# danijar/embodied

Hardware: AMD Instinct MI355X
Metric: env steps/sec + learner train-steps/sec, 64 envs 84x84x4 obs, 1/2/4/8 GPU (higher is better)
Workload: dtype u8

## Files before the change

### embodied_amd/csrc/device_util.h

```cpp
#pragma once

#include "kernels.h"

#include <cstdint>

namespace emb {
namespace {

typedef unsigned int u32x4 __attribute__((ext_vector_type(4)));

typedef __attribute__((address_space(1))) u32x4 gu32x4;
template <bool kNonTemporal>
__device__ __forceinline__ u32x4 load16(const u32x4* p) {
  const gu32x4* g = (const gu32x4*)p;
  if constexpr (kNonTemporal) return __builtin_nontemporal_load(g);
  else return *g;
}
template <bool kNonTemporal>
__device__ __forceinline__ void store16(u32x4* p, u32x4 v) {
  gu32x4* g = (gu32x4*)p;
  if constexpr (kNonTemporal) __builtin_nontemporal_store(v, g);
  else *g = v;
}

constexpr int kThreads = 256;

template <typename T>
__device__ __forceinline__ T gload(const void* p) {
  return *(const __attribute__((address_space(1))) T*)p;
}
template <typename T>
__device__ __forceinline__ void gstore(void* p, T v) {
  *(__attribute__((address_space(1))) T*)p = v;
}

template <typename T>
__device__ __forceinline__ void copy_unit(const uint8_t* s, uint8_t* d) {
  gstore<T>(d, gload<T>(s));
}

typedef unsigned int u32x2_t __attribute__((ext_vector_type(2)));

__device__ __forceinline__ void copy_bytes(const uint8_t* s, uint8_t* d, int unit) {
  switch (unit) {
    case 16: copy_unit<u32x4>(s, d); break;
    case 8: copy_unit<u32x2_t>(s, d); break;
    case 4: copy_unit<uint32_t>(s, d); break;
    case 2: copy_unit<uint16_t>(s, d); break;
    default: copy_unit<uint8_t>(s, d); break;
  }
}

template <typename T>
__device__ __forceinline__ T put_masked(const uint8_t* src, uint8_t* pool, uint8_t* out, bool keep) {
  const T v = gload<T>(src) * static_cast<T>(keep ? 1 : 0);
  if (pool) gstore<T>(pool, v);
  if (out) gstore<T>(out, v);
  return v;
}

__device__ __forceinline__ uint16_t put_masked_bf16(const uint8_t* src, uint8_t* pool, uint8_t* out, bool keep) {
  const float x = __uint_as_float(static_cast<uint32_t>(gload<uint16_t>(src)) << 16);
  const uint16_t v = static_cast<uint16_t>(__float_as_uint(x * (keep ? 1.f : 0.f)) >> 16);
  if (pool) gstore<uint16_t>(pool, v);
  if (out) gstore<uint16_t>(out, v);
  return v;
}

template <typename T>
__device__ __forceinline__ uint64_t masked_bits(T v) {
  static_assert(sizeof(T) <= 8, "a masked element fits 64 bits");
  uint64_t bits = 0;
  __builtin_memcpy(&bits, &v, sizeof(T));
  return bits;
}

__device__ __forceinline__ uint64_t put_masked_as(int dtype, const uint8_t* src, uint8_t* pool, uint8_t* out,
                                                  bool keep) {
  switch (dtype) {
    case kU8: case kBool: return masked_bits(put_masked<uint8_t>(src, pool, out, keep));
    case kI8: return masked_bits(put_masked<int8_t>(src, pool, out, keep));
    case kI16: return masked_bits(put_masked<int16_t>(src, pool, out, keep));
    case kI32: return masked_bits(put_masked<int32_t>(src, pool, out, keep));
    case kI64: return masked_bits(put_masked<int64_t>(src, pool, out, keep));
    case kF16: return masked_bits(put_masked<_Float16>(src, pool, out, keep));
    case kBF16: return masked_bits(put_masked_bf16(src, pool, out, keep));
    case kF32: return masked_bits(put_masked<float>(src, pool, out, keep));
    default: return masked_bits(put_masked<double>(src, pool, out, keep));
  }
}

int dtype_size(int dtype) {
  switch (dtype) {
    case kU8: case kI8: case kBool: return 1;
    case kI16: case kF16: case kBF16: return 2;
    case kI32: case kF32: return 4;
    case kI64: case kF64: return 8;
    default: return 0;
  }
}

}
}
```

### embodied_amd/csrc/step.hip

```cpp
#include "device_util.h"

#include <hip/hip_bf16.h>
#include <hip/hip_fp16.h>
#include <hip/hip_ext.h>

#include <algorithm>
#include <cstddef>
#include <cstring>

namespace emb {
namespace {


template <typename Out>
__device__ __forceinline__ Out cvt(uint8_t v, float scale, float offset);
template <> __device__ __forceinline__ uint8_t cvt<uint8_t>(uint8_t v, float, float) { return v; }
template <> __device__ __forceinline__ float cvt<float>(uint8_t v, float s, float o) { return fmaf(static_cast<float>(v), s, o); }
template <> __device__ __forceinline__ __half cvt<__half>(uint8_t v, float s, float o) { return __float2half(fmaf(static_cast<float>(v), s, o)); }
template <> __device__ __forceinline__ __hip_bfloat16 cvt<__hip_bfloat16>(uint8_t v, float s, float o) { return __float2bfloat16(fmaf(static_cast<float>(v), s, o)); }

template <typename Out>
struct alignas(4 * sizeof(Out)) Quad { Out v[4]; };

typedef unsigned int u32x2 __attribute__((ext_vector_type(2)));

template <typename Out>
__device__ __forceinline__ void store_quad(Out* dst, const Quad<Out>& q) {
  if constexpr (sizeof(Quad<Out>) == 4) {
    uint32_t w;
    __builtin_memcpy(&w, &q, 4);
    __builtin_nontemporal_store(w, reinterpret_cast<uint32_t*>(dst));
  } else if constexpr (sizeof(Quad<Out>) == 8) {
    u32x2 w;
    __builtin_memcpy(&w, &q, 8);
    __builtin_nontemporal_store(w, reinterpret_cast<u32x2*>(dst));
  } else {
    u32x4 w;
    __builtin_memcpy(&w, &q, 16);
    __builtin_nontemporal_store(w, reinterpret_cast<u32x4*>(dst));
  }
}

template <typename Out, int C, bool kChannelsFirst>
__global__ __launch_bounds__(kThreads) void obs_stack_kernel(
    const uint8_t* src, const int32_t* env_ids, Out* dst, int64_t pixels,
    float scale, float offset) {
  const int64_t n = blockIdx.y;
  const int64_t e = env_ids ? env_ids[n] : n;
  const int64_t quads = pixels >> 2;
  const uint32_t* frame = reinterpret_cast<const uint32_t*>(src + e * pixels * C);
  Out* out = dst + n * pixels * C;
  for (int64_t q = static_cast<int64_t>(blockIdx.x) * kThreads + threadIdx.x; q < quads;
       q += static_cast<int64_t>(gridDim.x) * kThreads) {
    uint32_t w[C];
#pragma unroll
    for (int c = 0; c < C; ++c) w[c] = frame[q * C + c];
    auto byte_at = [&w](int idx) {
      return static_cast<uint8_t>((w[idx >> 2] >> ((idx & 3) * 8)) & 0xFFu);
    };
    if (kChannelsFirst) {
#pragma unroll
      for (int c = 0; c < C; ++c) {
        Quad<Out> o;
#pragma unroll
        for (int p = 0; p < 4; ++p) o.v[p] = cvt<Out>(byte_at(p * C + c), scale, offset);
        store_quad(out + c * pixels + q * 4, o);
      }
    } else {
#pragma unroll
      for (int j = 0; j < C; ++j) {
        Quad<Out> o;
#pragma unroll
        for (int p = 0; p < 4; ++p) o.v[p] = cvt<Out>(byte_at(j * 4 + p), scale, offset);
        store_quad(out + (q * C + j) * 4, o);
      }
    }
  }
}

template <typename Out>
__global__ __launch_bounds__(kThreads) void obs_stack_generic_kernel(
    const uint8_t* src, const int32_t* env_ids, Out* dst, int64_t pixels,
    int64_t channels, int layout, float scale, float offset) {
  const int64_t n = blockIdx.y;
  const int64_t e = env_ids ? env_ids[n] : n;
  const int64_t elems = pixels * channels;
  const uint8_t* frame = src + e * elems;
  Out* out = dst + n * elems;
  for (int64_t i = static_cast<int64_t>(blockIdx.x) * kThreads + threadIdx.x; i < elems;
       i += static_cast<int64_t>(gridDim.x) * kThreads) {
    int64_t s = i;
    if (layout == kLayoutChannelsFirst) {
      const int64_t c = i / pixels, p = i - c * pixels;
      s = p * channels + c;
    }
    out[i] = cvt<Out>(frame[s], scale, offset);
  }
}

template <typename Out>
hipError_t obs_stack_typed(const uint8_t* src, const int32_t* env_ids, void* dst,
                           int64_t n, int64_t pixels, int64_t channels, int layout,
                           float scale, float offset, hipStream_t stream) {
  Out* out = static_cast<Out*>(dst);
  const bool fast = pixels % 4 == 0 && channels >= 1 && channels <= 4 &&
                    reinterpret_cast<uint64_t>(src) % 4 == 0 &&
                    (pixels * channels) % 4 == 0 &&
                    reinterpret_cast<uint64_t>(dst) % (4 * sizeof(Out)) == 0;
  if (!fast) {
    const int64_t elems = pixels * channels;
    dim3 grid(static_cast<uint32_t>(std::min<int64_t>((elems + kThreads - 1) / kThreads, 64)),
              static_cast<uint32_t>(n));
    hipLaunchKernelGGL(obs_stack_generic_kernel<Out>, grid, dim3(kThreads), 0, stream,
                       src, env_ids, out, pixels, channels, layout, scale, offset);
    return hipGetLastError();
  }
  const int64_t quads = pixels / 4;
  dim3 grid(static_cast<uint32_t>(std::min<int64_t>((quads + kThreads - 1) / kThreads, 32)),
            static_cast<uint32_t>(n));
  const bool cf = layout == kLayoutChannelsFirst && channels > 1;
#define EMB_OBS(C)                                                                         \
  if (cf) hipLaunchKernelGGL((obs_stack_kernel<Out, C, true>), grid, dim3(kThreads), 0,   \
                             stream, src, env_ids, out, pixels, scale, offset);           \
  else hipLaunchKernelGGL((obs_stack_kernel<Out, C, false>), grid, dim3(kThreads), 0,     \
                          stream, src, env_ids, out, pixels, scale, offset);
  switch (channels) {
    case 1: EMB_OBS(1) break;
    case 2: EMB_OBS(2) break;
    case 3: EMB_OBS(3) break;
    default: EMB_OBS(4) break;
  }
#undef EMB_OBS
  return hipGetLastError();
}

struct PreKey {
  const uint8_t* src;
  uint8_t* pool;
  int64_t rowbytes;
};
struct PreCarry {
  const uint8_t* src;
  uint8_t* pool;
  const uint8_t* flags;
  int32_t rowbytes, dtype, elem, pad;
};
struct alignas(16) PreTable {
  uint8_t* stepid_pool;
  int32_t* rows_out;
  PreKey narrow[kPreNarrow];
  PreCarry carry;
  uint32_t words[1];
};
struct PrewriteArgs {
  const uint8_t* frames;
  void* dst;
  uint8_t* frame_pool;
  int32_t pixels, frame_blocks;
  float scale, offset;
  int32_t n, n_narrow;
  const PreTable* table;
};
static_assert(sizeof(PrewriteArgs) == 56, "obs_stack_insert_kernel's arguments (passed one by one) fit the 14 preloaded dwords");

__device__ __forceinline__ void prewrite_carry(const PreTable& t, const uint32_t* tab, int32_t n_envs,
                                               int64_t n) {
  const PreCarry c = t.carry;
  if (!c.src) return;
  const int64_t prev = static_cast<int32_t>(gload<uint32_t>(tab + 6 * static_cast<int64_t>(n_envs) + n));
  const int64_t off = static_cast<int64_t>(threadIdx.x) * c.elem;
  if (prev < 0 || off >= c.rowbytes) return;
  const bool keep = gload<uint8_t>(c.flags + prev) == 0;
  const uint8_t* src = c.src + n * c.rowbytes + off;
  uint8_t* pool = c.pool + prev * c.rowbytes + off;
  put_masked_as(c.dtype, src, pool, nullptr, keep);
}

__device__ __forceinline__ void prewrite_narrow(const PrewriteArgs& a, int64_t n) {
  const PreTable& t = *a.table;
  const uint32_t* tab = t.words;
  prewrite_carry(t, tab, a.n, n);
  const int64_t row = static_cast<int32_t>(gload<uint32_t>(tab + n));
  if (row < 0) return;
  uint32_t sid = 0;
  if (threadIdx.x < kStepBytes / 4)
    sid = gload<uint32_t>(tab + a.n + n * (kStepBytes / 4) + threadIdx.x);
  PreKey key[kPreNarrow];
#pragma unroll
  for (int k = 0; k < kPreNarrow; ++k) key[k] = t.narrow[k];
  uint8_t v[kPreNarrow];
#pragma unroll
  for (int k = 0; k < kPreNarrow; ++k) {
    v[k] = 0;
    if (k < a.n_narrow && static_cast<int64_t>(threadIdx.x) < key[k].rowbytes)
      v[k] = gload<uint8_t>(key[k].src + n * key[k].rowbytes + threadIdx.x);
  }
#pragma unroll
  for (int k = 0; k < kPreNarrow; ++k)
    if (k < a.n_narrow && static_cast<int64_t>(threadIdx.x) < key[k].rowbytes)
      gstore<uint8_t>(key[k].pool + row * key[k].rowbytes + threadIdx.x, v[k]);
  if (t.stepid_pool && threadIdx.x < kStepBytes / 4)
    gstore<uint32_t>(t.stepid_pool + row * kStepBytes + threadIdx.x * 4, sid);
  if (t.rows_out && threadIdx.x == 0) t.rows_out[n] = static_cast<int32_t>(row);
}
static_assert(kThreads >= 256, "a narrow key (<= 256 bytes per step) is one byte per lane");

template <typename Out, int C, bool kChannelsFirst>
__global__ __launch_bounds__(kThreads) void obs_stack_insert_kernel(
    const uint8_t* frames, const PreTable* table, uint8_t* frame_pool, void* dst,
    int32_t pixels_, int32_t frame_blocks, int32_t n_envs, int32_t n_narrow, float scale, float offset) {
  const PrewriteArgs a{frames, dst, frame_pool, pixels_, frame_blocks, scale, offset, n_envs, n_narrow, table};
  if (blockIdx.x < static_cast<uint32_t>(n_envs)) {
    prewrite_narrow(a, blockIdx.x);
    return;
  }
  const uint32_t id = blockIdx.x - static_cast<uint32_t>(n_envs);
  const int64_t n = id / static_cast<uint32_t>(frame_blocks);
  const uint32_t block = id - static_cast<uint32_t>(n) * static_cast<uint32_t>(frame_blocks);
  const int64_t pixels = a.pixels;
  const int64_t quads = pixels >> 2;
  const uint32_t* frame = reinterpret_cast<const uint32_t*>(a.frames + n * pixels * C);
  Out* out = static_cast<Out*>(a.dst) + n * pixels * C;
  const int64_t row = static_cast<int32_t>(gload<uint32_t>(a.table->words + n));
  uint32_t* pool = reinterpret_cast<uint32_t*>(a.frame_pool + row * pixels * C);
  const int64_t stride = static_cast<int64_t>(frame_blocks) * kThreads;
  for (int64_t q = static_cast<int64_t>(block) * kThreads + threadIdx.x; q < quads; q += stride) {
    uint32_t w[C];
    if constexpr (C == 4) {
      const u32x4 v = __builtin_nontemporal_load(reinterpret_cast<const u32x4*>(frame) + q);
      w[0] = v[0]; w[1] = v[1]; w[2] = v[2]; w[3] = v[3];
    } else {
#pragma unroll
      for (int c = 0; c < C; ++c) w[c] = frame[q * C + c];
    }
    auto byte_at = [&w](int idx) {
      return static_cast<uint8_t>((w[idx >> 2] >> ((idx & 3) * 8)) & 0xFFu);
    };
    if (kChannelsFirst) {
#pragma unroll
      for (int c = 0; c < C; ++c) {
        Quad<Out> o;
#pragma unroll
        for (int p = 0; p < 4; ++p) o.v[p] = cvt<Out>(byte_at(p * C + c), a.scale, a.offset);
        store_quad(out + c * pixels + q * 4, o);
      }
    } else {
#pragma unroll
      for (int j = 0; j < C; ++j) {
        Quad<Out> o;
#pragma unroll
        for (int p = 0; p < 4; ++p) o.v[p] = cvt<Out>(byte_at(j * 4 + p), a.scale, a.offset);
        store_quad(out + (q * C + j) * 4, o);
      }
    }
    if (row >= 0) {
      if constexpr (C == 4) {
        __builtin_nontemporal_store(u32x4{w[0], w[1], w[2], w[3]}, reinterpret_cast<u32x4*>(pool) + q);
      } else {
#pragma unroll
        for (int c = 0; c < C; ++c) __builtin_nontemporal_store(w[c], pool + q * C + c);
      }
    }
  }
}

template <typename Out>
hipError_t obs_stack_insert_typed(const PrewriteArgs& a, int64_t channels, int layout,
                                  hipStream_t stream, hipEvent_t stop) {
  dim3 grid(static_cast<uint32_t>(a.n) * static_cast<uint32_t>(a.frame_blocks + 1));
  const bool cf = layout == kLayoutChannelsFirst && channels > 1;
#define EMB_PRE_ARGS a.frames, a.table, a.frame_pool, a.dst, a.pixels, a.frame_blocks, a.n, a.n_narrow, a.scale, a.offset
#define EMB_PRE(C)                                                                                \
  if (cf && stop) hipExtLaunchKernelGGL((obs_stack_insert_kernel<Out, C, true>), grid,            \
                                        dim3(kThreads), 0, stream, nullptr, stop, 0, EMB_PRE_ARGS); \
  else if (cf) hipLaunchKernelGGL((obs_stack_insert_kernel<Out, C, true>), grid, dim3(kThreads),  \
                                  0, stream, EMB_PRE_ARGS);                                       \
  else if (stop) hipExtLaunchKernelGGL((obs_stack_insert_kernel<Out, C, false>), grid,            \
                                       dim3(kThreads), 0, stream, nullptr, stop, 0, EMB_PRE_ARGS); \
  else hipLaunchKernelGGL((obs_stack_insert_kernel<Out, C, false>), grid, dim3(kThreads), 0,      \
                          stream, EMB_PRE_ARGS);
  switch (channels) {
    case 1: EMB_PRE(1) break;
    case 2: EMB_PRE(2) break;
    case 3: EMB_PRE(3) break;
    default: EMB_PRE(4) break;
  }
#undef EMB_PRE
#undef EMB_PRE_ARGS
  return hipGetLastError();
}

struct PublishArgs {
  const uint8_t* src;
  uint8_t* pool;
  uint8_t* out;
  const int32_t* rows;
  const uint8_t* flags;
  int32_t n, rowbytes, dtype, elem;
};
static_assert(sizeof(PublishArgs) <= 64, "publish_one_kernel's arguments are preloaded");

__global__ __launch_bounds__(kThreads) void publish_one_kernel(
    const uint8_t* src_, uint8_t* pool_, uint8_t* out_, const int32_t* rows, const uint8_t* flags,
    int32_t n, int32_t rowbytes, int32_t dtype, int32_t elem) {
  const PublishArgs a{src_, pool_, out_, rows, flags, n, rowbytes, dtype, elem};
  const int64_t epr = a.rowbytes / a.elem;
  const int64_t e = static_cast<int64_t>(blockIdx.x) * kThreads + threadIdx.x;
  if (e >= epr * a.n) return;
  const int64_t r = e / epr;
  const int64_t off = (e - r * epr) * a.elem;
  const int64_t row = a.rows[r];
  const bool by_row = (a.dtype & 0x100) != 0;
  const bool keep = !a.flags || (by_row ? row < 0 || gload<uint8_t>(a.flags + row) == 0
                                        : gload<uint8_t>(a.flags + r) == 0);
  const uint8_t* src = a.src + r * a.rowbytes + off;
  uint8_t* pool = row >= 0 ? a.pool + row * a.rowbytes + off : nullptr;
  uint8_t* out = a.out ? a.out + r * a.rowbytes + off : nullptr;
  put_masked_as(a.dtype & 0xFF, src, pool, out, keep);
}


__device__ __forceinline__ void notify_host(uint32_t* counter, uint32_t* flag, uint32_t seq) {
  if (!flag) return;
  __threadfence_system();
  __syncthreads();
  if (threadIdx.x == 0) {
    const uint32_t seen = __hip_atomic_fetch_add(counter, 1u, __ATOMIC_ACQ_REL, __HIP_MEMORY_SCOPE_AGENT);
    if (seen + 1 == gridDim.x) {
      __hip_atomic_store(counter, 0u, __ATOMIC_RELAXED, __HIP_MEMORY_SCOPE_AGENT);
      __threadfence_system();
      __hip_atomic_store(flag, seq, __ATOMIC_RELEASE, __HIP_MEMORY_SCOPE_SYSTEM);
    }
  }
}

template <typename T>
__global__ __launch_bounds__(kThreads) void mask_rows_kernel(
    const T* act, T* out, int64_t n, int64_t row_elems, const uint8_t* is_last, uint32_t* counter,
    uint32_t* flag, uint32_t seq) {
  const int64_t total = n * row_elems;
  for (int64_t i = static_cast<int64_t>(blockIdx.x) * kThreads + threadIdx.x; i < total;
       i += static_cast<int64_t>(gridDim.x) * kThreads) {
    const int64_t r = i / row_elems;
    out[i] = act[i] * static_cast<T>(is_last[r] ? 0 : 1);
  }
  notify_host(counter, flag, seq);
}

template <>
__global__ __launch_bounds__(kThreads) void mask_rows_kernel<__hip_bfloat16>(
    const __hip_bfloat16* act, __hip_bfloat16* out, int64_t n, int64_t row_elems,
    const uint8_t* is_last, uint32_t* counter, uint32_t* flag, uint32_t seq) {
  const int64_t total = n * row_elems;
  const uint16_t* bits = reinterpret_cast<const uint16_t*>(act);
  uint16_t* obits = reinterpret_cast<uint16_t*>(out);
  for (int64_t i = static_cast<int64_t>(blockIdx.x) * kThreads + threadIdx.x; i < total;
       i += static_cast<int64_t>(gridDim.x) * kThreads) {
    const float x = __uint_as_float(static_cast<uint32_t>(bits[i]) << 16);
    const float y = x * (is_last[i / row_elems] ? 0.f : 1.f);
    obits[i] = static_cast<uint16_t>(__float_as_uint(y) >> 16);
  }
  notify_host(counter, flag, seq);
}


__global__ __launch_bounds__(kThreads) void window_kernel(
    const uint8_t* src, uint8_t* dst, int64_t total, int64_t start, int64_t count,
    int64_t rowbytes, int unit, int64_t units_per_seq) {
  const int64_t b = blockIdx.y;
  const uint8_t* s = src + (b * total + start) * rowbytes;
  uint8_t* d = dst + b * count * rowbytes;
  for (int64_t u = static_cast<int64_t>(blockIdx.x) * kThreads + threadIdx.x;
       u < units_per_seq; u += static_cast<int64_t>(gridDim.x) * kThreads)
    copy_bytes(s + u * unit, d + u * unit, unit);
}

__global__ __launch_bounds__(kThreads) void copy_bytes_kernel(const uint8_t* __restrict__ src,
                                                             uint8_t* __restrict__ dst, int64_t bytes) {
  const bool aligned = ((reinterpret_cast<uintptr_t>(src) | reinterpret_cast<uintptr_t>(dst)) & 15) == 0;
  const int64_t vecs = aligned ? bytes >> 4 : 0;
  const int64_t stride = static_cast<int64_t>(gridDim.x) * kThreads;
  int64_t i = static_cast<int64_t>(blockIdx.x) * kThreads + threadIdx.x;
  for (; i + 3 * stride < vecs; i += 4 * stride) {
    const u32x4 a = reinterpret_cast<const u32x4*>(src)[i], b = reinterpret_cast<const u32x4*>(src)[i + stride];
    const u32x4 c = reinterpret_cast<const u32x4*>(src)[i + 2 * stride], d = reinterpret_cast<const u32x4*>(src)[i + 3 * stride];
    reinterpret_cast<u32x4*>(dst)[i] = a;
    reinterpret_cast<u32x4*>(dst)[i + stride] = b;
    reinterpret_cast<u32x4*>(dst)[i + 2 * stride] = c;
    reinterpret_cast<u32x4*>(dst)[i + 3 * stride] = d;
  }
  for (; i < vecs; i += stride) reinterpret_cast<u32x4*>(dst)[i] = reinterpret_cast<const u32x4*>(src)[i];
  for (int64_t j = (vecs << 4) + static_cast<int64_t>(blockIdx.x) * kThreads + threadIdx.x; j < bytes; j += stride)
    dst[j] = src[j];
}

}

hipError_t launch_window(const uint8_t* src, uint8_t* dst, int64_t batch, int64_t total,
                         int64_t start, int64_t count, int64_t rowbytes,
                         hipStream_t stream) {
  if (batch <= 0 || count <= 0) return hipSuccess;
  const uint64_t mix = reinterpret_cast<uint64_t>(src) | reinterpret_cast<uint64_t>(dst) |
                       static_cast<uint64_t>(rowbytes);
  const int unit = mix % 16 == 0 ? 16 : mix % 8 == 0 ? 8 : mix % 4 == 0 ? 4 : mix % 2 == 0 ? 2 : 1;
  const int64_t units = count * rowbytes / unit;
  const int64_t bx = std::min<int64_t>((units + kThreads - 1) / kThreads, 1024);
  hipLaunchKernelGGL(window_kernel, dim3(static_cast<uint32_t>(bx), static_cast<uint32_t>(batch)),
                     dim3(kThreads), 0, stream, src, dst, total, start, count, rowbytes, unit, units);
  return hipGetLastError();
}

hipError_t launch_copy_bytes(const void* src, void* dst, int64_t bytes, hipStream_t stream) {
  if (bytes <= 0) return hipSuccess;
  const int64_t blocks = std::max<int64_t>(1, std::min<int64_t>(256, ((bytes >> 4) + kThreads - 1) / kThreads));
  hipLaunchKernelGGL(copy_bytes_kernel, dim3(static_cast<uint32_t>(blocks)), dim3(kThreads), 0, stream,
                     static_cast<const uint8_t*>(src), static_cast<uint8_t*>(dst), bytes);
  return hipGetLastError();
}

hipError_t launch_mask_rows(const void* act, void* out, int64_t n, int64_t row_elems, int dtype,
                            const uint8_t* is_last, hipStream_t stream, uint32_t* counter, uint32_t* flag,
                            uint32_t seq) {
  const int64_t total = n * row_elems;
  if (total <= 0) return flag ? hipErrorInvalidValue : hipSuccess;
  const dim3 grid(static_cast<uint32_t>(std::min<int64_t>((total + kThreads - 1) / kThreads, 2048)));
#define EMB_MASK(T) hipLaunchKernelGGL(mask_rows_kernel<T>, grid, dim3(kThreads), 0, stream, static_cast<const T*>(act), static_cast<T*>(out), n, row_elems, is_last, counter, flag, seq)
  switch (dtype) {
    case kU8: case kBool: EMB_MASK(uint8_t); break;
    case kI8: EMB_MASK(int8_t); break;
    case kI16: EMB_MASK(int16_t); break;
    case kI32: EMB_MASK(int32_t); break;
    case kI64: EMB_MASK(int64_t); break;
    case kF16: EMB_MASK(_Float16); break;
    case kBF16: EMB_MASK(__hip_bfloat16); break;
    case kF32: EMB_MASK(float); break;
    case kF64: EMB_MASK(double); break;
    default: return hipErrorInvalidValue;
  }
#undef EMB_MASK
  return hipGetLastError();
}

hipError_t launch_publish_one(const void* src, void* pool, void* out, const int32_t* rows_dev,
                              const uint8_t* flags, int64_t n, int64_t rowbytes, int dtype,
                              hipStream_t stream, hipEvent_t stop, bool flags_by_row) {
  if (n <= 0 || rowbytes <= 0) return hipSuccess;
  PublishArgs a;
  a.src = static_cast<const uint8_t*>(src);
  a.pool = static_cast<uint8_t*>(pool);
  a.out = static_cast<uint8_t*>(out);
  a.rows = rows_dev;
  a.flags = flags;
  a.n = static_cast<int32_t>(n);
  a.rowbytes = static_cast<int32_t>(rowbytes);
  if (flags) {
    a.dtype = dtype | (flags_by_row ? 0x100 : 0);
    a.elem = dtype_size(dtype);
    if (a.elem == 0 || rowbytes % a.elem) return hipErrorInvalidValue;
  } else {
    a.dtype = kU8;
    a.elem = 1;
  }
  const int64_t elems = n * (rowbytes / a.elem);
  if (n > INT32_MAX || rowbytes > INT32_MAX) return hipErrorInvalidValue;
  const dim3 grid(static_cast<uint32_t>((elems + kThreads - 1) / kThreads));
  if (stop) hipExtLaunchKernelGGL(publish_one_kernel, grid, dim3(kThreads), 0, stream, nullptr, stop, 0,
                                  a.src, a.pool, a.out, a.rows, a.flags, a.n, a.rowbytes, a.dtype, a.elem);
  else hipLaunchKernelGGL(publish_one_kernel, grid, dim3(kThreads), 0, stream,
                          a.src, a.pool, a.out, a.rows, a.flags, a.n, a.rowbytes, a.dtype, a.elem);
  return hipGetLastError();
}

bool prewrite_supported(const PrewritePlan& p) {
  return p.n > 0 && p.n <= (1 << 24) && p.pixels > 0 && p.pixels <= INT32_MAX && p.pixels % 4 == 0 &&
         p.channels >= 1 && p.channels <= 4 &&
         reinterpret_cast<uint64_t>(p.frames) % 16 == 0 &&
         reinterpret_cast<uint64_t>(p.frame_pool) % 16 == 0 &&
         (p.pixels * p.channels) % 16 == 0 &&
         reinterpret_cast<uint64_t>(p.dst) % 16 == 0 && p.n_narrow >= 0 && p.n_narrow <= kPreNarrow &&
         (p.out_dtype == kU8 || p.out_dtype == kF16 || p.out_dtype == kBF16 || p.out_dtype == kF32);
}

size_t prewrite_table_bytes(int64_t n) {
  return offsetof(PreTable, words) + static_cast<size_t>(n) * 7 * sizeof(uint32_t);
}

void prewrite_fill_table(void* dst, const PrewritePlan& p, const int32_t* rows, const uint8_t* stepids) {
  PreTable head;
  head.stepid_pool = p.stepid_pool;
  head.rows_out = p.rows_out;
  for (int k = 0; k < kPreNarrow; ++k)
    head.narrow[k] = k < p.n_narrow ? PreKey{p.narrow[k].src, p.narrow[k].pool, p.narrow[k].rowbytes}
                                    : PreKey{nullptr, nullptr, 0};
  head.carry = PreCarry{nullptr, nullptr, nullptr, 0, 0, 1, 0};
  if (p.carry_src && p.carry_rows) {
    const int elem = dtype_size(p.carry_dtype);
    head.carry = PreCarry{p.carry_src, p.carry_pool, p.carry_flags, static_cast<int32_t>(p.carry_rowbytes),
                          p.carry_dtype, elem > 0 ? elem : 1, 0};
  }
  uint8_t* out = static_cast<uint8_t*>(dst);
  std::memcpy(out, &head, offsetof(PreTable, words));
  out += offsetof(PreTable, words);
  std::memcpy(out, rows, static_cast<size_t>(p.n) * sizeof(int32_t));
  out += static_cast<size_t>(p.n) * sizeof(int32_t);
  std::memcpy(out, stepids, static_cast<size_t>(p.n) * kStepBytes);
  out += static_cast<size_t>(p.n) * kStepBytes;
  if (head.carry.src) std::memcpy(out, p.carry_rows, static_cast<size_t>(p.n) * sizeof(int32_t));
}

bool carry_supported(int64_t rowbytes, int dtype) {
  const int elem = dtype_size(dtype);
  return elem > 0 && rowbytes > 0 && rowbytes % elem == 0 && rowbytes / elem <= kThreads &&
         rowbytes <= INT32_MAX;
}

hipError_t launch_obs_stack_insert(const PrewritePlan& p, hipStream_t stream, hipEvent_t stop) {
  if (!prewrite_supported(p) || !p.table_dev) return hipErrorInvalidValue;
  PrewriteArgs a;
  a.frames = p.frames;
  a.dst = p.dst;
  a.frame_pool = p.frame_pool;
  a.pixels = static_cast<int32_t>(p.pixels);
  a.frame_blocks = static_cast<int32_t>(std::min<int64_t>((p.pixels / 4 + kThreads - 1) / kThreads, 32));
  a.scale = p.scale;
  a.offset = p.offset;
  a.n = p.n;
  a.n_narrow = p.n_narrow;
  a.table = static_cast<const PreTable*>(p.table_dev);
  switch (p.out_dtype) {
    case kU8: return obs_stack_insert_typed<uint8_t>(a, p.channels, p.layout, stream, stop);
    case kF16: return obs_stack_insert_typed<__half>(a, p.channels, p.layout, stream, stop);
    case kBF16: return obs_stack_insert_typed<__hip_bfloat16>(a, p.channels, p.layout, stream, stop);
    default: return obs_stack_insert_typed<float>(a, p.channels, p.layout, stream, stop);
  }
}

hipError_t launch_obs_stack(const uint8_t* src, const int32_t* env_ids, void* dst, int64_t n,
                            int64_t pixels, int64_t channels, int layout, int out_dtype,
                            float scale, float offset, hipStream_t stream) {
  if (n <= 0 || pixels <= 0 || channels <= 0) return hipSuccess;
  switch (out_dtype) {
    case kU8: return obs_stack_typed<uint8_t>(src, env_ids, dst, n, pixels, channels, layout, scale, offset, stream);
    case kF16: return obs_stack_typed<__half>(src, env_ids, dst, n, pixels, channels, layout, scale, offset, stream);
    case kBF16: return obs_stack_typed<__hip_bfloat16>(src, env_ids, dst, n, pixels, channels, layout, scale, offset, stream);
    case kF32: return obs_stack_typed<float>(src, env_ids, dst, n, pixels, channels, layout, scale, offset, stream);
    default: return hipErrorInvalidValue;
  }
}

}
```

### embodied_amd/csrc/synth_env.hip

```cpp
#include "device_util.h"

#include <algorithm>
#include <cstring>

namespace emb {
namespace {


struct SynthArgs {
  int32_t* counters;
  const uint8_t* reset;
  uint8_t* image;
  float* reward;
  int32_t off_first, off_last, off_terminal;
  int32_t frame_bytes, env0, episode_len, n_turn;
};
static_assert(sizeof(SynthArgs) <= 64, "synth_env_kernel's arguments (passed one by one, n from the grid) are preloaded");

struct alignas(16) SynthMaskJob {
  const uint8_t* src;
  uint8_t* out;
  int32_t rowbytes, dtype, elem;
  int32_t off_first, off_last, off_terminal;
};
static_assert(sizeof(SynthMaskJob) == kSynthJobBytes, "kernels.h states the size of the block");

struct SynthStep {
  int32_t count;
  bool restart, done;
};

__device__ __forceinline__ SynthStep synth_step(const SynthArgs& a, int64_t e) {
  const int32_t n = a.n_turn >> 1, turn = a.n_turn & 1;
  const int32_t* __restrict__ in = a.counters + turn * 2 * n;
  int32_t count = in[2 * e];
  const bool was_done = in[2 * e + 1] != 0;
  const bool restart = (a.reset && a.reset[e]) || was_done;
  const int64_t length = a.episode_len + ((a.env0 + e) % 8) * 13;
  count = restart ? 0 : count + 1;
  return {count, restart, !restart && count >= length};
}

__device__ __forceinline__ void synth_frame(const SynthArgs& a, int64_t e, int32_t count, uint32_t blocks) {
  const uint32_t salt = static_cast<uint32_t>((a.env0 + e) * 131 + static_cast<int64_t>(count) * 7);
  u32x4* out = reinterpret_cast<u32x4*>(a.image + e * a.frame_bytes);
  const int64_t vecs = a.frame_bytes >> 4;
  auto word = [salt](int64_t byte0) {
    const uint32_t x = salt + static_cast<uint32_t>(byte0);
    return (x & 0xFF) | (((x + 1) & 0xFF) << 8) | (((x + 2) & 0xFF) << 16) | (((x + 3) & 0xFF) << 24);
  };
  for (int64_t i = static_cast<int64_t>(blockIdx.x) * kThreads + threadIdx.x; i < vecs;
       i += static_cast<int64_t>(blocks) * kThreads)
    __builtin_nontemporal_store(
        u32x4{word(i * 16), word(i * 16 + 4), word(i * 16 + 8), word(i * 16 + 12)}, out + i);
}

__device__ __forceinline__ uint64_t synth_masked_action(const SynthMaskJob& j, const uint8_t* reset, int64_t e) {
  const int64_t off = static_cast<int64_t>(threadIdx.x) * j.elem;
  if (!j.src || off >= j.rowbytes) return 0;
  const bool keep = !reset || gload<uint8_t>(reset + e) == 0;
  return put_masked_as(j.dtype, j.src + e * j.rowbytes + off, nullptr, j.out + e * j.rowbytes + off, keep);
}

__device__ __forceinline__ void synth_bookkeeping(const SynthArgs& a, int64_t e, const SynthStep& s,
                                                  uint8_t* is_first, uint8_t* is_last, uint8_t* is_terminal) {
  const int32_t n = a.n_turn >> 1, turn = a.n_turn & 1;
  int32_t* next = a.counters + (1 - turn) * 2 * n;
  next[2 * e] = s.count;
  next[2 * e + 1] = s.done ? 1 : 0;
  a.reward[e] = s.restart ? 0.f : static_cast<float>(s.count % 7);
  is_first[e] = s.restart ? 1 : 0;
  is_last[e] = s.done ? 1 : 0;
  is_terminal[e] = s.done ? 1 : 0;
}

__global__ __launch_bounds__(kThreads) void synth_env_kernel(
    int32_t* counters, const uint8_t* reset, uint8_t* image, float* reward, int32_t off_first,
    int32_t off_last, int32_t off_terminal, int32_t frame_bytes, int32_t env0, int32_t len_turn) {
  const SynthArgs a{counters, reset, image, reward, off_first, off_last, off_terminal,
                    frame_bytes, env0, len_turn & 0x7FFFFFFF,
                    static_cast<int32_t>(gridDim.y << 1 | (static_cast<uint32_t>(len_turn) >> 31))};
  const int64_t e = blockIdx.y;
  const SynthStep s = synth_step(a, e);
  synth_frame(a, e, s.count, gridDim.x);
  if (blockIdx.x == 0 && threadIdx.x == 0) {
    uint8_t* flags = reinterpret_cast<uint8_t*>(a.reward);
    synth_bookkeeping(a, e, s, flags + a.off_first, flags + a.off_last, flags + a.off_terminal);
  }
}

__global__ __launch_bounds__(kThreads) void synth_env_masked_kernel(
    int32_t* counters, const uint8_t* reset, uint8_t* image, float* reward,
    const SynthMaskJob* __restrict__ job, int32_t frame_bytes, int32_t env0, int32_t len_turn, int32_t n_envs) {
  const SynthArgs a{counters, reset, image, reward, 0, 0, 0,
                    frame_bytes & ~15, env0, len_turn & 0x7FFFFFFF,
                    static_cast<int32_t>(static_cast<uint32_t>(n_envs) << 1 | (static_cast<uint32_t>(len_turn) >> 31))};
  const uint32_t blocks = (static_cast<uint32_t>(frame_bytes) & 15u) + 1;
  const int64_t e = blockIdx.y;
  if (blockIdx.x != 0) {
    synth_frame(a, e, synth_step(a, e).count, blocks);
    return;
  }
  const SynthMaskJob j = *job;
  const SynthStep s = synth_step(a, e);
  synth_frame(a, e, s.count, blocks);
  synth_masked_action(j, a.reset, e);
  if (threadIdx.x == 0) {
    uint8_t* flags = reinterpret_cast<uint8_t*>(a.reward);
    synth_bookkeeping(a, e, s, flags + j.off_first, flags + j.off_last, flags + j.off_terminal);
  }
}

__global__ __launch_bounds__(kThreads) void synth_env_far_kernel(
    const SynthArgs a, uint8_t* is_first, uint8_t* is_last, uint8_t* is_terminal, const SynthMaskJob j) {
  const int64_t e = blockIdx.y;
  const SynthStep s = synth_step(a, e);
  synth_frame(a, e, s.count, gridDim.x);
  if (blockIdx.x == 0) {
    synth_masked_action(j, a.reset, e);
    if (threadIdx.x == 0) synth_bookkeeping(a, e, s, is_first, is_last, is_terminal);
  }
}

bool synth_args(SynthArgs* a, uint8_t* image, float* reward, int64_t n, int64_t frame_bytes, int64_t env0,
                int64_t episode_len, const uint8_t* reset, int32_t* counters, int turn, dim3* grid) {
  if (frame_bytes % 16 != 0 || reinterpret_cast<uint64_t>(image) % 16 != 0 || n > (1 << 29) ||
      frame_bytes > INT32_MAX || env0 > INT32_MAX || episode_len > INT32_MAX)
    return false;
  a->counters = counters;
  a->reset = reset;
  a->image = image;
  a->reward = reward;
  a->off_first = a->off_last = a->off_terminal = 0;
  a->frame_bytes = static_cast<int32_t>(frame_bytes);
  a->env0 = static_cast<int32_t>(env0);
  a->episode_len = static_cast<int32_t>(episode_len);
  a->n_turn = static_cast<int32_t>(n << 1 | (turn & 1));
  const int64_t vecs = frame_bytes >> 4;
  constexpr int64_t per_env = 4;
  const uint32_t gx = static_cast<uint32_t>(std::max<int64_t>(1, std::min<int64_t>(per_env, vecs / kThreads)));
  *grid = dim3(gx, static_cast<uint32_t>(n));
  return true;
}

bool synth_offsets(const float* reward, const uint8_t* is_first, const uint8_t* is_last,
                   const uint8_t* is_terminal, int32_t* of, int32_t* ol, int32_t* ot) {
  const int64_t base = reinterpret_cast<int64_t>(reward);
  const int64_t f = reinterpret_cast<int64_t>(is_first) - base, l = reinterpret_cast<int64_t>(is_last) - base,
                t = reinterpret_cast<int64_t>(is_terminal) - base;
  auto fits = [](int64_t x) { return x >= INT32_MIN && x <= INT32_MAX; };
  if (!fits(f) || !fits(l) || !fits(t)) return false;
  *of = static_cast<int32_t>(f);
  *ol = static_cast<int32_t>(l);
  *ot = static_cast<int32_t>(t);
  return true;
}

int32_t len_turn_word(const SynthArgs& a, int turn) {
  return static_cast<int32_t>(static_cast<uint32_t>(a.episode_len) | (static_cast<uint32_t>(turn & 1) << 31));
}

}

hipError_t launch_synth_env(uint8_t* image, float* reward, uint8_t* is_first, uint8_t* is_last,
                            uint8_t* is_terminal, int64_t n, int64_t frame_bytes, int64_t env0,
                            int64_t episode_len, const uint8_t* reset, int32_t* counters, int turn,
                            hipStream_t stream) {
  if (n <= 0) return hipSuccess;
  SynthArgs a;
  dim3 grid;
  if (!synth_args(&a, image, reward, n, frame_bytes, env0, episode_len, reset, counters, turn, &grid))
    return hipErrorInvalidValue;
  if (synth_offsets(reward, is_first, is_last, is_terminal, &a.off_first, &a.off_last, &a.off_terminal)) {
    hipLaunchKernelGGL(synth_env_kernel, grid, dim3(kThreads), 0, stream, a.counters, a.reset, a.image,
                       a.reward, a.off_first, a.off_last, a.off_terminal, a.frame_bytes, a.env0,
                       len_turn_word(a, turn));
  } else {
    hipLaunchKernelGGL(synth_env_far_kernel, grid, dim3(kThreads), 0, stream, a, is_first, is_last,
                       is_terminal, SynthMaskJob{nullptr, nullptr, 0, 0, 1, 0, 0, 0});
  }
  return hipGetLastError();
}

bool synth_mask_job(void* job, const void* act, void* masked_out, int64_t rowbytes, int dtype,
                    const float* reward, const uint8_t* is_first, const uint8_t* is_last,
                    const uint8_t* is_terminal) {
  SynthMaskJob j{static_cast<const uint8_t*>(act), static_cast<uint8_t*>(masked_out),
                 static_cast<int32_t>(rowbytes), dtype, std::max(dtype_size(dtype), 1), 0, 0, 0};
  const bool near = synth_offsets(reward, is_first, is_last, is_terminal, &j.off_first, &j.off_last,
                                  &j.off_terminal);
  std::memcpy(job, &j, sizeof(j));
  return near;
}

hipError_t launch_synth_env_masked(uint8_t* image, float* reward, uint8_t* is_first, uint8_t* is_last,
                                   uint8_t* is_terminal, int64_t n, int64_t frame_bytes, int64_t env0,
                                   int64_t episode_len, const uint8_t* reset, int32_t* counters, int turn,
                                   const void* job_host, const void* job_dev, hipStream_t stream) {
  if (n <= 0) return hipSuccess;
  SynthMaskJob j;
  std::memcpy(&j, job_host, sizeof(j));
  if (!j.src || !j.out || !carry_supported(j.rowbytes, j.dtype) || j.elem != dtype_size(j.dtype))
    return hipErrorInvalidValue;
  SynthArgs a;
  dim3 grid;
  if (!synth_args(&a, image, reward, n, frame_bytes, env0, episode_len, reset, counters, turn, &grid))
    return hipErrorInvalidValue;
  if (job_dev) {
    hipLaunchKernelGGL(synth_env_masked_kernel, grid, dim3(kThreads), 0, stream, a.counters, a.reset, a.image,
                       a.reward, static_cast<const SynthMaskJob*>(job_dev),
                       a.frame_bytes | static_cast<int32_t>(grid.x - 1), a.env0,
                       len_turn_word(a, turn), static_cast<int32_t>(n));
  } else {
    hipLaunchKernelGGL(synth_env_far_kernel, grid, dim3(kThreads), 0, stream, a, is_first, is_last,
                       is_terminal, j);
  }
  return hipGetLastError();
}

}
```

Baseline: 5.425 million.

## Hoist and batch dependent loads in prewrite and masked synth kernels

Reorders the narrow-key prewrite and the masked synthetic-env kernel so that all table, counter, reset and action loads are issued up front. Scheduling barriers and register pins keep the loads grouped, so their latencies overlap instead of forming serial load chains. Action element size and count are packed into spare bits of the scalar kernel arguments, and the reward pointer moves into the job struct. This adds launch constraints (reset must be non-null and episode length below 2^23, otherwise the far kernel runs) and packs grid.x-1 into 2 bits instead of 4, which could break for larger grids.

```diff
diff --git a/embodied_amd/csrc/device_util.h b/embodied_amd/csrc/device_util.h
--- a/embodied_amd/csrc/device_util.h
+++ b/embodied_amd/csrc/device_util.h
@@ -52,16 +52,25 @@
 }
 
 template <typename T>
+__device__ __forceinline__ T masked_mul(T x, bool keep) {
+  return x * static_cast<T>(keep ? 1 : 0);
+}
+
+__device__ __forceinline__ uint16_t masked_mul_bf16(uint16_t bits, bool keep) {
+  const float x = __uint_as_float(static_cast<uint32_t>(bits) << 16);
+  return static_cast<uint16_t>(__float_as_uint(x * (keep ? 1.f : 0.f)) >> 16);
+}
+
+template <typename T>
 __device__ __forceinline__ T put_masked(const uint8_t* src, uint8_t* pool, uint8_t* out, bool keep) {
-  const T v = gload<T>(src) * static_cast<T>(keep ? 1 : 0);
+  const T v = masked_mul(gload<T>(src), keep);
   if (pool) gstore<T>(pool, v);
   if (out) gstore<T>(out, v);
   return v;
 }
 
 __device__ __forceinline__ uint16_t put_masked_bf16(const uint8_t* src, uint8_t* pool, uint8_t* out, bool keep) {
-  const float x = __uint_as_float(static_cast<uint32_t>(gload<uint16_t>(src)) << 16);
-  const uint16_t v = static_cast<uint16_t>(__float_as_uint(x * (keep ? 1.f : 0.f)) >> 16);
+  const uint16_t v = masked_mul_bf16(gload<uint16_t>(src), keep);
   if (pool) gstore<uint16_t>(pool, v);
   if (out) gstore<uint16_t>(out, v);
   return v;
@@ -90,6 +99,46 @@
   }
 }
 
+__device__ __forceinline__ uint64_t load_elem(int elem, const uint8_t* src, bool on) {
+  uint32_t b1 = 0, b2 = 0, b4 = 0;
+  uint64_t b8 = 0;
+  if (on & (elem == 1)) b1 = gload<uint8_t>(src);
+  if (on & (elem == 2)) b2 = gload<uint16_t>(src);
+  if (on & (elem == 4)) b4 = gload<uint32_t>(src);
+  if (on & (elem == 8)) b8 = gload<uint64_t>(src);
+  return b8 | (b1 | b2 | b4);
+}
+
+__device__ __forceinline__ void store_elem(int elem, uint8_t* dst, uint64_t bits) {
+  switch (elem) {
+    case 1: gstore<uint8_t>(dst, static_cast<uint8_t>(bits)); break;
+    case 2: gstore<uint16_t>(dst, static_cast<uint16_t>(bits)); break;
+    case 4: gstore<uint32_t>(dst, static_cast<uint32_t>(bits)); break;
+    default: gstore<uint64_t>(dst, bits); break;
+  }
+}
+
+template <typename T>
+__device__ __forceinline__ uint64_t masked_bits_of(uint64_t bits, bool keep) {
+  T x;
+  __builtin_memcpy(&x, &bits, sizeof(T));
+  return masked_bits(masked_mul(x, keep));
+}
+
+__device__ __forceinline__ uint64_t mask_elem_as(int dtype, uint64_t bits, bool keep) {
+  switch (dtype) {
+    case kU8: case kBool: return masked_bits_of<uint8_t>(bits, keep);
+    case kI8: return masked_bits_of<int8_t>(bits, keep);
+    case kI16: return masked_bits_of<int16_t>(bits, keep);
+    case kI32: return masked_bits_of<int32_t>(bits, keep);
+    case kI64: return masked_bits_of<int64_t>(bits, keep);
+    case kF16: return masked_bits_of<_Float16>(bits, keep);
+    case kBF16: return masked_bits(masked_mul_bf16(static_cast<uint16_t>(bits), keep));
+    case kF32: return masked_bits_of<float>(bits, keep);
+    default: return masked_bits_of<double>(bits, keep);
+  }
+}
+
 int dtype_size(int dtype) {
   switch (dtype) {
     case kU8: case kI8: case kBool: return 1;
diff --git a/embodied_amd/csrc/step.hip b/embodied_amd/csrc/step.hip
--- a/embodied_amd/csrc/step.hip
+++ b/embodied_amd/csrc/step.hip
@@ -163,51 +163,69 @@
 };
 static_assert(sizeof(PrewriteArgs) == 56, "obs_stack_insert_kernel's arguments (passed one by one) fit the 14 preloaded dwords");
 
-__device__ __forceinline__ void prewrite_carry(const PreTable& t, const uint32_t* tab, int32_t n_envs,
-                                               int64_t n) {
-  const PreCarry c = t.carry;
-  if (!c.src) return;
-  const int64_t prev = static_cast<int32_t>(gload<uint32_t>(tab + 6 * static_cast<int64_t>(n_envs) + n));
-  const int64_t off = static_cast<int64_t>(threadIdx.x) * c.elem;
-  if (prev < 0 || off >= c.rowbytes) return;
-  const bool keep = gload<uint8_t>(c.flags + prev) == 0;
-  const uint8_t* src = c.src + n * c.rowbytes + off;
-  uint8_t* pool = c.pool + prev * c.rowbytes + off;
-  put_masked_as(c.dtype, src, pool, nullptr, keep);
+template <typename T>
+__device__ __forceinline__ void pin(T& x) {
+  asm volatile("" : "+s"(x));
+}
+template <typename T>
+__device__ __forceinline__ void pin_lane(T& x) {
+  asm volatile("" : "+v"(x));
 }
 
 __device__ __forceinline__ void prewrite_narrow(const PrewriteArgs& a, int64_t n) {
   const PreTable& t = *a.table;
   const uint32_t* tab = t.words;
-  prewrite_carry(t, tab, a.n, n);
-  const int64_t row = static_cast<int32_t>(gload<uint32_t>(tab + n));
-  if (row < 0) return;
+  const int64_t lane = threadIdx.x;
+  const bool sid_lane = lane < kStepBytes / 4;
   uint32_t sid = 0;
-  if (threadIdx.x < kStepBytes / 4)
-    sid = gload<uint32_t>(tab + a.n + n * (kStepBytes / 4) + threadIdx.x);
+  if (sid_lane) sid = gload<uint32_t>(tab + a.n + n * (kStepBytes / 4) + lane);
+  int32_t row32 = static_cast<int32_t>(gload<uint32_t>(tab + n));
+  int32_t prev32 = static_cast<int32_t>(gload<uint32_t>(tab + 6 * static_cast<int64_t>(a.n) + n));
+  PreCarry c = t.carry;
   PreKey key[kPreNarrow];
 #pragma unroll
   for (int k = 0; k < kPreNarrow; ++k) key[k] = t.narrow[k];
-  uint8_t v[kPreNarrow];
+  uint8_t* stepid_pool = t.stepid_pool;
+  int32_t* rows_out = t.rows_out;
+  __builtin_amdgcn_sched_barrier(0);
+  pin(c.src); pin(c.pool); pin(c.flags); pin(c.rowbytes); pin(c.dtype); pin(c.elem);
+#pragma unroll
+  for (int k = 0; k < kPreNarrow; ++k) { pin(key[k].src); pin(key[k].pool); pin(key[k].rowbytes); }
+  pin(stepid_pool); pin(rows_out); pin(row32); pin(prev32);
+  const int64_t row = row32, prev = prev32;
+  const int64_t coff = lane * c.elem;
+  const bool carried = (c.src != nullptr) & (prev >= 0) & (coff < c.rowbytes);
+  const bool placed = row >= 0;
+  const uint64_t act = load_elem(c.elem, c.src + n * c.rowbytes + coff, carried);
+  bool live[kPreNarrow];
+  uint32_t v[kPreNarrow];
 #pragma unroll
   for (int k = 0; k < kPreNarrow; ++k) {
+    live[k] = placed & (k < a.n_narrow) & (lane < key[k].rowbytes);
     v[k] = 0;
-    if (k < a.n_narrow && static_cast<int64_t>(threadIdx.x) < key[k].rowbytes)
-      v[k] = gload<uint8_t>(key[k].src + n * key[k].rowbytes + threadIdx.x);
-  }
+    if (live[k]) v[k] = gload<uint8_t>(key[k].src + n * key[k].rowbytes + lane);
+  }
+  uint32_t last = 0;
+  if (carried) last = gload<uint8_t>(c.flags + prev);
+  __builtin_amdgcn_sched_barrier(0);
+  uint64_t act_bits = act;
+  pin_lane(sid); pin_lane(act_bits); pin_lane(last);
+#pragma unroll
+  for (int k = 0; k < kPreNarrow; ++k) pin_lane(v[k]);
+  if (carried)
+    store_elem(c.elem, c.pool + prev * c.rowbytes + coff, mask_elem_as(c.dtype, act_bits, last == 0));
 #pragma unroll
   for (int k = 0; k < kPreNarrow; ++k)
-    if (k < a.n_narrow && static_cast<int64_t>(threadIdx.x) < key[k].rowbytes)
-      gstore<uint8_t>(key[k].pool + row * key[k].rowbytes + threadIdx.x, v[k]);
-  if (t.stepid_pool && threadIdx.x < kStepBytes / 4)
-    gstore<uint32_t>(t.stepid_pool + row * kStepBytes + threadIdx.x * 4, sid);
-  if (t.rows_out && threadIdx.x == 0) t.rows_out[n] = static_cast<int32_t>(row);
+    if (live[k]) gstore<uint8_t>(key[k].pool + row * key[k].rowbytes + lane, static_cast<uint8_t>(v[k]));
+  if (placed & (stepid_pool != nullptr) & sid_lane)
+    gstore<uint32_t>(stepid_pool + row * kStepBytes + lane * 4, sid);
+  if (placed & (rows_out != nullptr) & (lane == 0)) gstore<int32_t>(rows_out + n, static_cast<int32_t>(row));
 }
 static_assert(kThreads >= 256, "a narrow key (<= 256 bytes per step) is one byte per lane");
 
 template <typename Out, int C, bool kChannelsFirst>
 __global__ __launch_bounds__(kThreads) void obs_stack_insert_kernel(
-    const uint8_t* frames, const PreTable* table, uint8_t* frame_pool, void* dst,
+    const uint8_t* frames, const PreTable* __restrict__ table, uint8_t* frame_pool, void* dst,
     int32_t pixels_, int32_t frame_blocks, int32_t n_envs, int32_t n_narrow, float scale, float offset) {
   const PrewriteArgs a{frames, dst, frame_pool, pixels_, frame_blocks, scale, offset, n_envs, n_narrow, table};
   if (blockIdx.x < static_cast<uint32_t>(n_envs)) {
diff --git a/embodied_amd/csrc/synth_env.hip b/embodied_amd/csrc/synth_env.hip
--- a/embodied_amd/csrc/synth_env.hip
+++ b/embodied_amd/csrc/synth_env.hip
@@ -20,6 +20,7 @@
 struct alignas(16) SynthMaskJob {
   const uint8_t* src;
   uint8_t* out;
+  float* reward;
   int32_t rowbytes, dtype, elem;
   int32_t off_first, off_last, off_terminal;
 };
@@ -29,16 +30,19 @@
   int32_t count;
   bool restart, done;
 };
+
+__device__ __forceinline__ SynthStep synth_advance(const SynthArgs& a, int64_t e, int32_t count, bool restart) {
+  const int64_t length = a.episode_len + ((a.env0 + e) % 8) * 13;
+  count = restart ? 0 : count + 1;
+  return {count, restart, !restart && count >= length};
+}
 
 __device__ __forceinline__ SynthStep synth_step(const SynthArgs& a, int64_t e) {
   const int32_t n = a.n_turn >> 1, turn = a.n_turn & 1;
   const int32_t* __restrict__ in = a.counters + turn * 2 * n;
   int32_t count = in[2 * e];
   const bool was_done = in[2 * e + 1] != 0;
-  const bool restart = (a.reset && a.reset[e]) || was_done;
-  const int64_t length = a.episode_len + ((a.env0 + e) % 8) * 13;
-  count = restart ? 0 : count + 1;
-  return {count, restart, !restart && count >= length};
+  return synth_advance(a, e, count, (a.reset && a.reset[e]) || was_done);
 }
 
 __device__ __forceinline__ void synth_frame(const SynthArgs& a, int64_t e, int32_t count, uint32_t blocks) {
@@ -89,26 +93,51 @@
   }
 }
 
+constexpr int32_t kSynthMaskedMaxLen = 1 << 23;
+template <typename T>
+__device__ __forceinline__ void pin(T& x) {
+  asm volatile("" : "+s"(x));
+}
+template <typename T>
+__device__ __forceinline__ void pin_lane(T& x) {
+  asm volatile("" : "+v"(x));
+}
 __global__ __launch_bounds__(kThreads) void synth_env_masked_kernel(
-    int32_t* counters, const uint8_t* reset, uint8_t* image, float* reward,
+    int32_t* counters, const uint8_t* reset, uint8_t* image, const uint8_t* act,
     const SynthMaskJob* __restrict__ job, int32_t frame_bytes, int32_t env0, int32_t len_turn, int32_t n_envs) {
-  const SynthArgs a{counters, reset, image, reward, 0, 0, 0,
-                    frame_bytes & ~15, env0, len_turn & 0x7FFFFFFF,
-                    static_cast<int32_t>(static_cast<uint32_t>(n_envs) << 1 | (static_cast<uint32_t>(len_turn) >> 31))};
-  const uint32_t blocks = (static_cast<uint32_t>(frame_bytes) & 15u) + 1;
+  SynthArgs a{counters, reset, image, nullptr, 0, 0, 0,
+              frame_bytes & ~15, env0, len_turn & (kSynthMaskedMaxLen - 1),
+              static_cast<int32_t>(static_cast<uint32_t>(n_envs) << 1 | (static_cast<uint32_t>(len_turn) >> 31))};
+  const uint32_t blocks = (static_cast<uint32_t>(frame_bytes) & 3u) + 1;
   const int64_t e = blockIdx.y;
   if (blockIdx.x != 0) {
     synth_frame(a, e, synth_step(a, e).count, blocks);
     return;
   }
-  const SynthMaskJob j = *job;
-  const SynthStep s = synth_step(a, e);
+  const int elem = 1 << ((frame_bytes >> 2) & 3);
+  const int64_t elems = ((static_cast<uint32_t>(len_turn) >> 23) & 0xFFu) + 1;
+  const bool lane_on = static_cast<int64_t>(threadIdx.x) < elems;
+  const int64_t off = (e * elems + threadIdx.x) * elem;
+  uint64_t raw = load_elem(elem, act + off, lane_on);
+  const int32_t* __restrict__ in = a.counters + (a.n_turn & 1) * 2 * (a.n_turn >> 1);
+  int32_t count = in[2 * e], done_word = in[2 * e + 1];
+  uint32_t reset_word = gload<uint8_t>(a.reset + e);
+  SynthMaskJob j = *job;
+  __builtin_amdgcn_sched_barrier(0);
+  count = __builtin_amdgcn_readfirstlane(count);
+  done_word = __builtin_amdgcn_readfirstlane(done_word);
+  reset_word = __builtin_amdgcn_readfirstlane(reset_word);
+  pin(j.out); pin(j.reward); pin(j.dtype); pin(j.off_first); pin(j.off_last); pin(j.off_terminal);
+  pin_lane(raw);
+  const bool was_done = done_word != 0, reset_e = reset_word != 0;
+  const SynthStep s = synth_advance(a, e, count, reset_e | was_done);
+  if (lane_on) store_elem(elem, j.out + off, mask_elem_as(j.dtype, raw, !reset_e));
+  if (threadIdx.x == 0) {
+    a.reward = j.reward;
+    uint8_t* flags = reinterpret_cast<uint8_t*>(j.reward);
+    synth_bookkeeping(a, e, s, flags + j.off_first, flags + j.off_last, flags + j.off_terminal);
+  }
   synth_frame(a, e, s.count, blocks);
-  synth_masked_action(j, a.reset, e);
-  if (threadIdx.x == 0) {
-    uint8_t* flags = reinterpret_cast<uint8_t*>(a.reward);
-    synth_bookkeeping(a, e, s, flags + j.off_first, flags + j.off_last, flags + j.off_terminal);
-  }
 }
 
 __global__ __launch_bounds__(kThreads) void synth_env_far_kernel(
@@ -177,7 +206,7 @@
                        len_turn_word(a, turn));
   } else {
     hipLaunchKernelGGL(synth_env_far_kernel, grid, dim3(kThreads), 0, stream, a, is_first, is_last,
-                       is_terminal, SynthMaskJob{nullptr, nullptr, 0, 0, 1, 0, 0, 0});
+                       is_terminal, SynthMaskJob{nullptr, nullptr, nullptr, 0, 0, 1, 0, 0, 0});
   }
   return hipGetLastError();
 }
@@ -185,7 +214,7 @@
 bool synth_mask_job(void* job, const void* act, void* masked_out, int64_t rowbytes, int dtype,
                     const float* reward, const uint8_t* is_first, const uint8_t* is_last,
                     const uint8_t* is_terminal) {
-  SynthMaskJob j{static_cast<const uint8_t*>(act), static_cast<uint8_t*>(masked_out),
+  SynthMaskJob j{static_cast<const uint8_t*>(act), static_cast<uint8_t*>(masked_out), const_cast<float*>(reward),
                  static_cast<int32_t>(rowbytes), dtype, std::max(dtype_size(dtype), 1), 0, 0, 0};
   const bool near = synth_offsets(reward, is_first, is_last, is_terminal, &j.off_first, &j.off_last,
                                   &j.off_terminal);
@@ -206,11 +235,13 @@
   dim3 grid;
   if (!synth_args(&a, image, reward, n, frame_bytes, env0, episode_len, reset, counters, turn, &grid))
     return hipErrorInvalidValue;
-  if (job_dev) {
+  if (job_dev && reset && episode_len < kSynthMaskedMaxLen) {
+    const int32_t elem_log2 = j.elem == 1 ? 0 : j.elem == 2 ? 1 : j.elem == 4 ? 2 : 3;
+    const int32_t elems = j.rowbytes / j.elem;
     hipLaunchKernelGGL(synth_env_masked_kernel, grid, dim3(kThreads), 0, stream, a.counters, a.reset, a.image,
-                       a.reward, static_cast<const SynthMaskJob*>(job_dev),
-                       a.frame_bytes | static_cast<int32_t>(grid.x - 1), a.env0,
-                       len_turn_word(a, turn), static_cast<int32_t>(n));
+                       j.src, static_cast<const SynthMaskJob*>(job_dev),
+                       a.frame_bytes | elem_log2 << 2 | static_cast<int32_t>(grid.x - 1), a.env0,
+                       len_turn_word(a, turn) | (elems - 1) << 23, static_cast<int32_t>(n));
   } else {
     hipLaunchKernelGGL(synth_env_far_kernel, grid, dim3(kThreads), 0, stream, a, is_first, is_last,
                        is_terminal, j);
```

After: 5.412 million. About the same (-0.2%).
